# anuragranj/cc

Measured on NVIDIA H100. Metric: train-step triplets/sec at 256x832x6lvl, higher is better.
Workload: dtype f32

## Files before the change

### cc_b200/csrc/conv_tc.cu

```cuda
#include "conv.cuh"

#ifndef CCB_CPU_SIM

#include <cuda.h>
#include <cudaTypedefs.h>

namespace ccb {

constexpr int TC_M = 128;
constexpr int TC_NMAX = 128;
constexpr int TC_KC = 8;
constexpr int TC_MAX_STAGES = 4;
constexpr int TC_PRODUCERS = 128;
constexpr int TC_CONSUMER_WARPS = 8;
constexpr int TC_THREADS = TC_PRODUCERS + 32 * TC_CONSUMER_WARPS;
constexpr int TC_MAX_TAPS = 49;
constexpr int TC_PRODUCER_REGS = 72, TC_CONSUMER_REGS = 216;

struct TcArgs {
    CUtensorMap wmap;
    const float* x;
    const float* bias;
    const float* res;
    float* out;
// ... 43 lines not shown
    }
}
__device__ __forceinline__ void fence_proxy_async() { asm volatile("fence.proxy.async.shared::cta;" ::: "memory"); }
__device__ __forceinline__ void fence_barrier_init() { asm volatile("fence.mbarrier_init.release.cluster;" ::: "memory"); }
__device__ __forceinline__ void mbar_arrive_expect_tx(uint64_t* bar, uint32_t bytes) {
    asm volatile("mbarrier.arrive.expect_tx.shared::cta.b64 _, [%0], %1;" ::"r"(smem_u32(bar)), "r"(bytes) : "memory");
}
__device__ __forceinline__ void tma_load_3d(void* dst, const CUtensorMap* map, uint64_t* bar, int c0, int c1, int c2) {
    asm volatile(
        "cp.async.bulk.tensor.3d.shared::cluster.global.mbarrier::complete_tx::bytes [%0], [%1, {%3, %4, %5}], [%2];"
        ::"r"(smem_u32(dst)), "l"(map), "r"(smem_u32(bar)), "r"(c0), "r"(c1), "r"(c2)
        : "memory");
}
__device__ __forceinline__ void tma_prefetch_map(const CUtensorMap* map) {
    asm volatile("prefetch.tensormap [%0];" ::"l"(map) : "memory");
}
__device__ __forceinline__ void cp_async_4(uint32_t dst, const float* src, bool valid) {
    asm volatile("cp.async.ca.shared.global [%0], [%1], 4, %2;" ::"r"(dst), "l"(src), "r"(valid ? 4 : 0) : "memory");
}
__device__ __forceinline__ void cp_async_arrive(uint64_t* bar) {
    asm volatile("cp.async.mbarrier.arrive.noinc.shared::cta.b64 [%0];" ::"r"(smem_u32(bar)) : "memory");
}
__device__ __forceinline__ void cp_async_wait_all() { asm volatile("cp.async.wait_all;" ::: "memory"); }
__device__ __forceinline__ float tf32_hi(float x) {
    uint32_t r;
    asm("cvt.rna.tf32.f32 %0, %1;" : "=r"(r) : "f"(x));
    return __uint_as_float(r);
}

__device__ __forceinline__ uint64_t wg_desc(uint32_t saddr) {
    return (uint64_t)((saddr & 0x3FFFF) >> 4) | ((uint64_t)1 << 16) | ((uint64_t)(1024 >> 4) << 32) | ((uint64_t)1 << 62);
}
__device__ __forceinline__ void wg_fence() { asm volatile("wgmma.fence.sync.aligned;" ::: "memory"); }
__device__ __forceinline__ void wg_commit() { asm volatile("wgmma.commit_group.sync.aligned;" ::: "memory"); }
template <int PENDING>
__device__ __forceinline__ void wg_wait() { asm volatile("wgmma.wait_group.sync.aligned %0;" ::"n"(PENDING) : "memory"); }
template <int R>
__device__ __forceinline__ void wg_fence_regs(float (&d)[R]) {
#pragma unroll
    for (int i = 0; i < R; ++i) asm volatile("" : "+f"(d[i])::"memory");
}
template <int K, int R>
__device__ __forceinline__ void wg_fence_regs(uint32_t (&d)[K][R]) {
#pragma unroll
    for (int k = 0; k < K; ++k)
#pragma unroll
        for (int i = 0; i < R; ++i) asm volatile("" : "+r"(d[k][i])::"memory");
}

__device__ __forceinline__ void wgmma_tf32_n16(float (&d)[8], uint64_t da, uint64_t db) {
    asm volatile(
        "{\n\t.reg .pred p;\n\tsetp.ne.b32 p, 1, 0;\n\t"
        "wgmma.mma_async.sync.aligned.m64n16k8.f32.tf32.tf32 "
        "{%0, %1, %2, %3, %4, %5, %6, %7}, "
        "%8, %9, p, 1, 1;\n\t}"
        : "+f"(d[0]), "+f"(d[1]), "+f"(d[2]), "+f"(d[3]), "+f"(d[4]), "+f"(d[5]), "+f"(d[6]), "+f"(d[7])
        : "l"(da), "l"(db));
}
__device__ __forceinline__ void wgmma_tf32_n32(float (&d)[16], uint64_t da, uint64_t db) {
    asm volatile(
        "{\n\t.reg .pred p;\n\tsetp.ne.b32 p, 1, 0;\n\t"
        "wgmma.mma_async.sync.aligned.m64n32k8.f32.tf32.tf32 "
        "{%0, %1, %2, %3, %4, %5, %6, %7, %8, %9, %10, %11, %12, %13, %14, %15}, "
        "%16, %17, p, 1, 1;\n\t}"
        : "+f"(d[0]), "+f"(d[1]), "+f"(d[2]), "+f"(d[3]), "+f"(d[4]), "+f"(d[5]), "+f"(d[6]), "+f"(d[7]),
          "+f"(d[8]), "+f"(d[9]), "+f"(d[10]), "+f"(d[11]), "+f"(d[12]), "+f"(d[13]), "+f"(d[14]), "+f"(d[15])
        : "l"(da), "l"(db));
}
__device__ __forceinline__ void wgmma_tf32_n64(float (&d)[32], uint64_t da, uint64_t db) {
    asm volatile(
        "{\n\t.reg .pred p;\n\tsetp.ne.b32 p, 1, 0;\n\t"
        "wgmma.mma_async.sync.aligned.m64n64k8.f32.tf32.tf32 "
        "{%0, %1, %2, %3, %4, %5, %6, %7, %8, %9, %10, %11, %12, %13, %14, %15,"
        " %16, %17, %18, %19, %20, %21, %22, %23, %24, %25, %26, %27, %28, %29, %30, %31}, "
        "%32, %33, p, 1, 1;\n\t}"
        : "+f"(d[0]), "+f"(d[1]), "+f"(d[2]), "+f"(d[3]), "+f"(d[4]), "+f"(d[5]), "+f"(d[6]), "+f"(d[7]),
          "+f"(d[8]), "+f"(d[9]), "+f"(d[10]), "+f"(d[11]), "+f"(d[12]), "+f"(d[13]), "+f"(d[14]), "+f"(d[15]),
          "+f"(d[16]), "+f"(d[17]), "+f"(d[18]), "+f"(d[19]), "+f"(d[20]), "+f"(d[21]), "+f"(d[22]), "+f"(d[23]),
          "+f"(d[24]), "+f"(d[25]), "+f"(d[26]), "+f"(d[27]), "+f"(d[28]), "+f"(d[29]), "+f"(d[30]), "+f"(d[31])
        : "l"(da), "l"(db));
}
__device__ __forceinline__ void wgmma_tf32_n128(float (&d)[64], uint64_t da, uint64_t db) {
    asm volatile(
        "{\n\t.reg .pred p;\n\tsetp.ne.b32 p, 1, 0;\n\t"
        "wgmma.mma_async.sync.aligned.m64n128k8.f32.tf32.tf32 "
        "{%0, %1, %2, %3, %4, %5, %6, %7, %8, %9, %10, %11, %12, %13, %14, %15,"
        " %16, %17, %18, %19, %20, %21, %22, %23, %24, %25, %26, %27, %28, %29, %30, %31,"
        " %32, %33, %34, %35, %36, %37, %38, %39, %40, %41, %42, %43, %44, %45, %46, %47,"
        " %48, %49, %50, %51, %52, %53, %54, %55, %56, %57, %58, %59, %60, %61, %62, %63}, "
        "%64, %65, p, 1, 1;\n\t}"
        : "+f"(d[0]), "+f"(d[1]), "+f"(d[2]), "+f"(d[3]), "+f"(d[4]), "+f"(d[5]), "+f"(d[6]), "+f"(d[7]),
          "+f"(d[8]), "+f"(d[9]), "+f"(d[10]), "+f"(d[11]), "+f"(d[12]), "+f"(d[13]), "+f"(d[14]), "+f"(d[15]),
          "+f"(d[16]), "+f"(d[17]), "+f"(d[18]), "+f"(d[19]), "+f"(d[20]), "+f"(d[21]), "+f"(d[22]), "+f"(d[23]),
          "+f"(d[24]), "+f"(d[25]), "+f"(d[26]), "+f"(d[27]), "+f"(d[28]), "+f"(d[29]), "+f"(d[30]), "+f"(d[31]),
          "+f"(d[32]), "+f"(d[33]), "+f"(d[34]), "+f"(d[35]), "+f"(d[36]), "+f"(d[37]), "+f"(d[38]), "+f"(d[39]),
          "+f"(d[40]), "+f"(d[41]), "+f"(d[42]), "+f"(d[43]), "+f"(d[44]), "+f"(d[45]), "+f"(d[46]), "+f"(d[47]),
          "+f"(d[48]), "+f"(d[49]), "+f"(d[50]), "+f"(d[51]), "+f"(d[52]), "+f"(d[53]), "+f"(d[54]), "+f"(d[55]),
          "+f"(d[56]), "+f"(d[57]), "+f"(d[58]), "+f"(d[59]), "+f"(d[60]), "+f"(d[61]), "+f"(d[62]), "+f"(d[63])
        : "l"(da), "l"(db));
}
template <int NT>
__device__ __forceinline__ void wgmma_tf32(float (&d)[NT / 2], uint64_t da, uint64_t db) {
    if constexpr (NT == 16) wgmma_tf32_n16(d, da, db);
    else if constexpr (NT == 32) wgmma_tf32_n32(d, da, db);
    else if constexpr (NT == 64) wgmma_tf32_n64(d, da, db);
    else wgmma_tf32_n128(d, da, db);
}

__device__ __forceinline__ void wgmma_tf32_rs_n16(float (&d)[8], const uint32_t (&a)[4], uint64_t db) {
    asm volatile(
        "{\n\t.reg .pred p;\n\tsetp.ne.b32 p, 1, 0;\n\t"
        "wgmma.mma_async.sync.aligned.m64n16k8.f32.tf32.tf32 "
        "{%0, %1, %2, %3, %4, %5, %6, %7}, "
        "{%8, %9, %10, %11}, %12, p, 1, 1;\n\t}"
        : "+f"(d[0]), "+f"(d[1]), "+f"(d[2]), "+f"(d[3]), "+f"(d[4]), "+f"(d[5]), "+f"(d[6]), "+f"(d[7])
        : "r"(a[0]), "r"(a[1]), "r"(a[2]), "r"(a[3]), "l"(db));
}
__device__ __forceinline__ void wgmma_tf32_rs_n32(float (&d)[16], const uint32_t (&a)[4], uint64_t db) {
    asm volatile(
        "{\n\t.reg .pred p;\n\tsetp.ne.b32 p, 1, 0;\n\t"
        "wgmma.mma_async.sync.aligned.m64n32k8.f32.tf32.tf32 "
        "{%0, %1, %2, %3, %4, %5, %6, %7, %8, %9, %10, %11, %12, %13, %14, %15}, "
        "{%16, %17, %18, %19}, %20, p, 1, 1;\n\t}"
        : "+f"(d[0]), "+f"(d[1]), "+f"(d[2]), "+f"(d[3]), "+f"(d[4]), "+f"(d[5]), "+f"(d[6]), "+f"(d[7]),
          "+f"(d[8]), "+f"(d[9]), "+f"(d[10]), "+f"(d[11]), "+f"(d[12]), "+f"(d[13]), "+f"(d[14]), "+f"(d[15])
        : "r"(a[0]), "r"(a[1]), "r"(a[2]), "r"(a[3]), "l"(db));
}
__device__ __forceinline__ void wgmma_tf32_rs_n64(float (&d)[32], const uint32_t (&a)[4], uint64_t db) {
    asm volatile(
// ... 70 lines not shown
    __device__ __forceinline__ void publish(int s) const { fence_proxy_async(); mbar_arrive(&full[s]); }
};

__device__ __forceinline__ TcRing tc_ring(int depth, int b_tile_bytes, int full_arrivals) {
    CCB_PDL_TRIGGER();
    extern __shared__ __align__(1024) unsigned char smem_raw[];
    unsigned char* smem = smem_raw + ((1024u - (smem_u32(smem_raw) & 1023u)) & 1023u);
    const int stage_bytes = 2 * TC_TILE_BYTES + 2 * b_tile_bytes;
    uint64_t* full = (uint64_t*)(smem + depth * stage_bytes);
    const TcRing r = {smem, depth, stage_bytes, b_tile_bytes, full, full + TC_MAX_STAGES};
    if (threadIdx.x == 0) {
        for (int s = 0; s < depth; ++s) { mbar_init(&r.full[s], full_arrivals); mbar_init(&r.empty[s], TC_CONSUMER_WARPS); }
        fence_barrier_init();
    }
    __syncthreads();
    CCB_PDL_SYNC();
    return r;
}

__device__ __forceinline__ int tc_acc_row(int wg, int wq, int lane, int half) { return wg * 64 + wq * 16 + (lane >> 2) + half * 8; }
__device__ __forceinline__ int tc_acc_col(int lane, int i, int e) { return 8 * i + 2 * (lane & 3) + e; }
__device__ __forceinline__ int tc_acc_reg(int i, int half, int e) { return 4 * i + 2 * half + e; }

template <int NT>
__device__ __forceinline__ void tc_consume(const TcRing& ring, int nkt, int wg, int lane, float (&acc)[NT / 2]) {
    float part[NT / 2];
#pragma unroll
    for (int j = 0; j < NT / 2; ++j) acc[j] = 0.f;
    const uint32_t base = smem_u32(ring.smem);
    for (int it = 0; it < nkt; ++it) {
        const int s = it % ring.depth;
        mbar_wait(&ring.full[s], (it / ring.depth) & 1);
        const TcTiles<uint32_t> t = ring.tiles(base, s);
        const uint32_t a_hi = t.a_hi + wg * (TC_TILE_BYTES / 2), a_lo = t.a_lo + wg * (TC_TILE_BYTES / 2);
#pragma unroll
        for (int j = 0; j < NT / 2; ++j) part[j] = 0.f;
        wg_fence();
#pragma unroll
        for (int ks = 0; ks < TC_KC / 2; ++ks) {
            const uint32_t koff = (uint32_t)ks * 32u;
            wgmma_tf32<NT>(part, wg_desc(a_lo + koff), wg_desc(t.b_hi + koff));
            wgmma_tf32<NT>(part, wg_desc(a_hi + koff), wg_desc(t.b_lo + koff));
        }
#pragma unroll
        for (int ks = 0; ks < TC_KC / 2; ++ks) {
            const uint32_t koff = (uint32_t)ks * 32u;
            wgmma_tf32<NT>(part, wg_desc(a_hi + koff), wg_desc(t.b_hi + koff));
        }
        wg_commit();
        wg_wait<0>();
        wg_fence_regs(part);
        if (lane == 0) mbar_arrive(&ring.empty[s]);
#pragma unroll
        for (int j = 0; j < NT / 2; ++j) acc[j] += part[j];
    }
}

struct TcAFrag { uint32_t hi[TC_KC / 2][4], lo[TC_KC / 2][4]; };

__device__ __forceinline__ int tc_a_idx(int r, int k) { return k * TC_M + (r ^ (8 * (k & 3))); }
__device__ __forceinline__ int tc_a_off(int r0, int t) { return tc_a_idx(r0, t) * 4; }
__device__ __forceinline__ void tc_load_a(const unsigned char* tile, int off, float (&v)[2][8]) {
#pragma unroll
    for (int h = 0; h < 2; ++h)
#pragma unroll
        for (int j = 0; j < 8; ++j) v[h][j] = *(const float*)(tile + ((off ^ (32 * h)) + 2048 * j));
}
__device__ __forceinline__ void tc_split_a(const float (&v)[2][8], TcAFrag& f) {
#pragma unroll
    for (int ks = 0; ks < TC_KC / 2; ++ks)
#pragma unroll
        for (int i = 0; i < 4; ++i) {
            const float x = v[i & 1][2 * ks + (i >> 1)], h = tf32_hi(x);
            f.hi[ks][i] = __float_as_uint(h);
            f.lo[ks][i] = __float_as_uint(tf32_hi(x - h));
        }
}

template <int NT>
__device__ __forceinline__ void tc_consume_rs(const TcRing& ring, int g, int nkt, int wg, int wq, int lane, float (&acc)[NT / 2]) {
    constexpr bool split_ahead = NT < 128;
    float part[NT / 2];
#pragma unroll
    for (int j = 0; j < NT / 2; ++j) acc[j] = 0.f;
    const uint32_t base = smem_u32(ring.smem);
    const int a_off = tc_a_off(wg * 64 + wq * 16 + (lane >> 2), lane & 3);
    TcAFrag cur, nxt;
    float v[2][8];
    int s = g % ring.depth;
    uint32_t phase = (g / ring.depth) & 1;
    if constexpr (split_ahead) {
        if (nkt > 0) {
            mbar_wait(&ring.full[s], phase);
            tc_load_a(ring.tiles(ring.smem, s).a_hi, a_off, v);
            tc_split_a(v, cur);
        }
    }
    for (int it = 0; it < nkt; ++it) {
        if constexpr (!split_ahead) {
            mbar_wait(&ring.full[s], phase);
            tc_load_a(ring.tiles(ring.smem, s).a_hi, a_off, v);
            tc_split_a(v, cur);
        }
        const TcTiles<uint32_t> tl = ring.tiles(base, s);
#pragma unroll
        for (int j = 0; j < NT / 2; ++j) part[j] = 0.f;
        wg_fence();
#pragma unroll
        for (int ks = 0; ks < TC_KC / 2; ++ks) {
            const uint32_t koff = (uint32_t)ks * 32u;
            wgmma_tf32_rs<NT>(part, cur.lo[ks], wg_desc(tl.b_hi + koff));
            wgmma_tf32_rs<NT>(part, cur.hi[ks], wg_desc(tl.b_lo + koff));
        }
#pragma unroll
        for (int ks = 0; ks < TC_KC / 2; ++ks)
            wgmma_tf32_rs<NT>(part, cur.hi[ks], wg_desc(tl.b_hi + (uint32_t)ks * 32u));
        wg_commit();
        const int s1 = s + 1 == ring.depth ? 0 : s + 1;
        const uint32_t phase1 = phase ^ (s1 == 0);
        if constexpr (split_ahead) {
            if (it + 1 < nkt) {
                mbar_wait(&ring.full[s1], phase1);
                tc_load_a(ring.tiles(ring.smem, s1).a_hi, a_off, v);
                tc_split_a(v, nxt);
            }
        }
        wg_wait<0>();
        wg_fence_regs(part);
        wg_fence_regs(cur.hi);
        wg_fence_regs(cur.lo);
        if (lane == 0) mbar_arrive(&ring.empty[s]);
#pragma unroll
        for (int j = 0; j < NT / 2; ++j) acc[j] += part[j];
        if constexpr (split_ahead) cur = nxt;
        s = s1;
        phase = phase1;
    }
}

struct TcUnit { int m0, n0, z, kt_beg, nkt; };
__device__ __forceinline__ TcUnit tc_unit(const TcArgs& a, int u) {
    TcUnit w;
    w.m0 = (u % a.tiles_m) * TC_M;
    u /= a.tiles_m;
    w.n0 = (u % a.tiles_n) * TC_NMAX;
    w.z = u / a.tiles_n;
    w.kt_beg = w.z * a.kt_per_split;
    w.nkt = max(0, min(a.ktiles, w.kt_beg + a.kt_per_split) - w.kt_beg);
    return w;
}

template <int NT>
__global__ void __launch_bounds__(TC_THREADS, 1) conv_tc_kernel(const __grid_constant__ TcArgs a) {
    const TcRing ring = tc_ring(a.depth, a.b_tile_bytes, TC_PRODUCERS + 1);
    const int tid = threadIdx.x, warp = tid >> 5, lane = tid & 31;
    const long long HWin = (long long)a.Hin * a.Win;

    if (warp < TC_PRODUCERS / 32) {
        wg_regs_dec<TC_PRODUCER_REGS>();
        const int r = tid;
        const int cpt = a.cpad >> 2;
        const int nchunks = a.ntaps * cpt;
        if (r == 0) tma_prefetch_map(&a.wmap);
        int g = 0;
// ... 18 lines not shown
                if (r == 0) {
                    mbar_arrive_expect_tx(&ring.full[s], 2 * ring.b_tile_bytes);
                    tma_load_3d(t.b_hi, &a.wmap, &ring.full[s], kt * (TC_KC * 4), w.n0, 0);
                    tma_load_3d(t.b_lo, &a.wmap, &ring.full[s], kt * (TC_KC * 4), w.n0, 1);
                }
                const uint32_t at = smem_u32(t.a_hi);
                const int q0 = kt * TC_KC;
                const int tap0 = q0 / cpt, c40 = q0 - tap0 * cpt;
                if (c40 + TC_KC <= cpt) {
                    bool ok = mvalid && tap0 < a.ntaps;
                    int pix = 0;
                    if (ok) {
                        const int iy = iy0 + a.off_y[tap0], ix = ix0 + a.off_x[tap0];
                        ok = (iy >= 0) && (iy < a.Hin) && (ix >= 0) && (ix < a.Win);
                        pix = iy * a.Win + ix;
                    }
                    const float* p = ok ? xb + (long long)(c40 * 4) * HWin + pix : a.x;
                    const int nv = ok ? (a.Cin - c40 * 4) : 0;
#pragma unroll
                    for (int c = 0; c < TC_KC; ++c)
#pragma unroll
                        for (int j = 0; j < 4; ++j) {
                            const bool v = c * 4 + j < nv;
                            cp_async_4(at + 4 * tc_a_idx(r, 4 * c + j), v ? p + (c * 4 + j) * HWin : a.x, v);
                        }
                } else {
                    int q = q0, tap = tap0, c4 = c40;
#pragma unroll
                    for (int c = 0; c < TC_KC; ++c) {
                        const float* p = a.x;
                        int nv = 0;
                        if (mvalid && q < nchunks) {
                            const int iy = iy0 + a.off_y[tap], ix = ix0 + a.off_x[tap];
                            if (iy >= 0 && iy < a.Hin && ix >= 0 && ix < a.Win) {
                                p = xb + (long long)(c4 * 4) * HWin + (iy * a.Win + ix);
                                nv = a.Cin - c4 * 4;
                            }
                        }
#pragma unroll
                        for (int j = 0; j < 4; ++j) {
                            const bool v = j < nv;
                            cp_async_4(at + 4 * tc_a_idx(r, 4 * c + j), v ? p + j * HWin : a.x, v);
                        }
                        ++q;
                        if (++c4 == cpt) { c4 = 0; ++tap; }
                    }
                }
                cp_async_arrive(&ring.full[s]);
            }
        }
        cp_async_wait_all();
    } else {
        wg_regs_inc<TC_CONSUMER_REGS>();
        const int wg = (warp - TC_PRODUCERS / 32) >> 2, wq = warp & 3;
        const long long HWout = (long long)a.Hout * a.Wout;
        int g = 0;
        for (int u = blockIdx.x; u < a.units; u += gridDim.x) {
            const TcUnit w = tc_unit(a, u);
            const int ntile = min(TC_NMAX, a.Ntot - w.n0);
            float acc[NT / 2];
            tc_consume_rs<NT>(ring, g, w.nkt, wg, wq, lane, acc);
            g += w.nkt;
#pragma unroll
            for (int half = 0; half < 2; ++half) {
                const int em = w.m0 + tc_acc_row(wg, wq, lane, half);
                if (em >= a.M) continue;
                int hw = a.Hc * a.Wc;
                int eb = em / hw;
                int rem = em - eb * hw;
                int eoy = rem / a.Wc, eox = rem - eoy * a.Wc;
                const long long obase = (long long)eb * a.Ntot * HWout + (long long)(eoy * a.out_stride + a.out_oy) * a.Wout +
                                        (eox * a.out_stride + a.out_ox);
#pragma unroll
                for (int i = 0; i < NT / 8; ++i)
#pragma unroll
                    for (int e = 0; e < 2; ++e) {
                        const int nl = tc_acc_col(lane, i, e);
                        if (nl < ntile) {
                            float o = acc[tc_acc_reg(i, half, e)];
                            const int n = w.n0 + nl;
                            const long long off = obase + (long long)n * HWout;
                            if (a.splits > 1) {
                                a.partial[(long long)w.z * a.out_numel + off] = o;
                            } else {
// ... 9 lines not shown
}

static int roundup(int v, int m) { return (v + m - 1) / m * m; }
static int tc_kp(int ntaps, int Cc) { return ntaps > 0 ? roundup(ntaps * roundup(Cc, 4), TC_KC * 4) : TC_KC * 4; }

static void tc_geometry(int N, int& nt, int& b_tile_bytes, int& depth, int& smem) {
    const int ntile_max = N < TC_NMAX ? N : TC_NMAX;
    nt = 16;
    while (nt < ntile_max) nt <<= 1;
    b_tile_bytes = nt * 128;
    const int stage = 2 * TC_TILE_BYTES + 2 * b_tile_bytes;
    depth = (TC_SMEM_MAX - 2048) / stage;
    if (depth > TC_MAX_STAGES) depth = TC_MAX_STAGES;
    smem = depth * stage + 2048;
}

template <typename Args>
static int tc_launch_kernel(void (*const (&kfns)[4])(const Args), const Args& a, int nt, dim3 grid, int smem, cudaStream_t st,
                            const char* what) {
    auto kfn = kfns[nt == 16 ? 0 : nt == 32 ? 1 : nt == 64 ? 2 : 3];
    cudaFuncSetAttribute(kfn, cudaFuncAttributeMaxDynamicSharedMemorySize, TC_SMEM_MAX);
    CCB_LAUNCH(kfn, grid, dim3(TC_THREADS), smem, st, a);
    return check_launch(what);
}

static void (*const TC_FPROP_KERNELS[4])(const TcArgs) = {conv_tc_kernel<16>, conv_tc_kernel<32>, conv_tc_kernel<64>,
                                                          conv_tc_kernel<128>};

static int tc_weight_map(CUtensorMap* map, const float* wp, int N, int Kp, int nt) {
    static PFN_cuTensorMapEncodeTiled_v12000 encode = [] {
        void* fn = nullptr;
        cudaDriverEntryPointQueryResult q;
        if (cudaGetDriverEntryPointByVersion("cuTensorMapEncodeTiled", &fn, 12000, cudaEnableDefault, &q) != cudaSuccess ||
            q != cudaDriverEntryPointSuccess)
            fn = nullptr;
        return (PFN_cuTensorMapEncodeTiled_v12000)fn;
    }();
    CCB_REQUIRE(encode, CCB_ERR_LAUNCH, "conv_tc: the driver has no cuTensorMapEncodeTiled");
    const cuuint64_t dims[3] = {(cuuint64_t)Kp, (cuuint64_t)N, 2};
    const cuuint64_t strides[2] = {(cuuint64_t)Kp * sizeof(float), (cuuint64_t)N * Kp * sizeof(float)};
    const cuuint32_t box[3] = {TC_KC * 4, (cuuint32_t)nt, 1};
    const cuuint32_t estrides[3] = {1, 1, 1};
    const CUresult rc = encode(map, CU_TENSOR_MAP_DATA_TYPE_FLOAT32, 3, (void*)wp, dims, strides, box, estrides,
                               CU_TENSOR_MAP_INTERLEAVE_NONE, CU_TENSOR_MAP_SWIZZLE_128B, CU_TENSOR_MAP_L2_PROMOTION_L2_256B,
                               CU_TENSOR_MAP_FLOAT_OOB_FILL_NONE);
    CCB_REQUIRE(rc == CUDA_SUCCESS, CCB_ERR_LAUNCH, "conv_tc: cuTensorMapEncodeTiled failed (%d) for N %d Kp %d", (int)rc, N, Kp);
// ... 4 lines not shown
                     float* wp, float* partial, int splits, cudaStream_t st) {
    a.cpad = roundup(Cc, 4);
    a.Kp = tc_kp(a.ntaps, Cc);
    WPrepDesc p;
    memset(&p, 0, sizeof(p));
    p.w = w; p.wp = wp; p.N = N; p.Cc = Cc; p.KK = KK; p.ntaps = a.ntaps; p.Kp = a.Kp; p.mode = mode; p.Ci = Ci;
    p.layout = WPREP_TC; p.p0 = a.cpad;
    for (int t = 0; t < a.ntaps; ++t) p.tap_index[t] = tap_index[t];
    const float* wpp = nullptr;
    int rc = wprep_get(p, st, &wpp);
    if (rc) return rc;
    a.Ntot = N;
    a.splits = splits;
    a.ktiles = a.Kp / (TC_KC * 4);
    a.kt_per_split = cdiv(a.ktiles, splits);
    a.partial = partial;
    int nt, smem;
    tc_geometry(N, nt, a.b_tile_bytes, a.depth, smem);
    rc = tc_weight_map(&a.wmap, wpp, N, a.Kp, nt);
    if (rc) return rc;
    a.tiles_m = cdiv(a.M, TC_M);
    a.tiles_n = cdiv(N, TC_NMAX);
    a.units = a.tiles_m * a.tiles_n * splits;
    static int sms = [] {
        int dev = 0, n = 0;
        cudaGetDevice(&dev);
        cudaDeviceGetAttribute(&n, cudaDevAttrMultiProcessorCount, dev);
        return n > 0 ? n : NUM_SMS;
    }();
    return tc_launch_kernel(TC_FPROP_KERNELS, a, nt, dim3(a.units < sms ? a.units : sms), smem, st, "conv_tc");
}

struct TcWgradArgs {
    const float* x;
    const float* dy;
    float* out;
    int B, Ci, Hi, Wi, Co, Ho, Wo, kh, kw, stride, pad;
    int cpad, Mtot;
    int P;
    int ktiles, kt_per_split, splits;
    int depth, b_tile_bytes;
};

template <int NT>
__global__ void __launch_bounds__(TC_THREADS, 1) conv_tc_wgrad_kernel(const TcWgradArgs a) {
    const TcRing ring = tc_ring(a.depth, a.b_tile_bytes, TC_PRODUCERS);
    const int tid = threadIdx.x, warp = tid >> 5, lane = tid & 31;
    const int m0 = blockIdx.x * TC_M, n0 = blockIdx.y * TC_NMAX;
    const int ntile = min(TC_NMAX, a.Co - n0);
    const int kt_beg = blockIdx.z * a.kt_per_split;
    const int nkt = min(a.ktiles, kt_beg + a.kt_per_split) - kt_beg;
    const int KK = a.kh * a.kw;
    const int HWo = a.Ho * a.Wo, HWi = a.Hi * a.Wi;

    if (warp < TC_PRODUCERS / 32) {
        const int c = tid & 7, rbase = tid >> 3;
        int rowoff[8], dky[8], dkx[8];
        unsigned rvalid = 0;
#pragma unroll
        for (int j = 0; j < 8; ++j) {
            int m = m0 + rbase + 16 * j;
            rowoff[j] = 0; dky[j] = dkx[j] = 0;
            if (m < a.Mtot) {
                int tap = m / a.cpad, ci = m - tap * a.cpad;
                if (ci < a.Ci) {
                    int ky = tap / a.kw, kx = tap - ky * a.kw;
                    dky[j] = ky - a.pad; dkx[j] = kx - a.pad;
                    rowoff[j] = ci * HWi + dky[j] * a.Wi + dkx[j];
                    rvalid |= 1u << j;
                }
            }
        }
        for (int it = 0; it < nkt; ++it) {
            const int s = it % ring.depth;
            const int p0 = ((kt_beg + it) * TC_KC + c) * 4;
            const bool pvalid = p0 < a.P;
            int b = 0, oy = 0, ox0 = 0;
            if (pvalid) {
                b = p0 / HWo;
                int rem = p0 - b * HWo;
                oy = rem / a.Wo;
                ox0 = rem - oy * a.Wo;
            }
            const float* xpix = a.x + (long long)b * a.Ci * HWi + (oy * a.stride) * a.Wi + ox0 * a.stride;
            const int iyb = oy * a.stride, ixb = ox0 * a.stride;
            float av[8][4];
            float4 bv[8];
#pragma unroll
            for (int j = 0; j < 8; ++j) {
                av[j][0] = av[j][1] = av[j][2] = av[j][3] = 0.f;
                const int iy = iyb + dky[j], ix0 = ixb + dkx[j];
                if (pvalid && ((rvalid >> j) & 1u) && iy >= 0 && iy < a.Hi) {
                    const float* px = xpix + rowoff[j];
                    if (ix0 >= 0 && ix0 + 3 * a.stride < a.Wi) {
#pragma unroll
                        for (int e = 0; e < 4; ++e) av[j][e] = __ldg(px + e * a.stride);
                    } else {
#pragma unroll
                        for (int e = 0; e < 4; ++e) {
                            const int ix = ix0 + e * a.stride;
                            if (ix >= 0 && ix < a.Wi) av[j][e] = __ldg(px + e * a.stride);
                        }
                    }
                }
                bv[j] = make_float4(0.f, 0.f, 0.f, 0.f);
                const int n = rbase + 16 * j;
                if (pvalid && n < ntile)
                    bv[j] = __ldg((const float4*)(a.dy + ((long long)b * a.Co + n0 + n) * HWo + oy * a.Wo + ox0));
            }
            const TcTiles<unsigned char*> t = ring.acquire(it, s);
#pragma unroll
            for (int j = 0; j < 8; ++j) {
                const int r = rbase + 16 * j, idx = tile_idx(r, c);
                tc_split_store(t.a_hi, t.a_lo, idx, make_float4(av[j][0], av[j][1], av[j][2], av[j][3]));
                if (r < NT) tc_split_store(t.b_hi, t.b_lo, idx, bv[j]);
            }
            ring.publish(s);
        }
    } else {
        const int wg = (warp - TC_PRODUCERS / 32) >> 2, wq = warp & 3;
        float acc[NT / 2];
        tc_consume<NT>(ring, nkt, wg, lane, acc);
        float* outp = a.out + (long long)blockIdx.z * a.Co * a.Ci * KK;
#pragma unroll
        for (int half = 0; half < 2; ++half) {
            const int em = m0 + tc_acc_row(wg, wq, lane, half);
            if (em >= a.Mtot) continue;
            const int etap = em / a.cpad;
            const int eci = em - etap * a.cpad;
            if (eci >= a.Ci) continue;
#pragma unroll
            for (int i = 0; i < NT / 8; ++i)
#pragma unroll
                for (int e = 0; e < 2; ++e) {
                    const int nl = tc_acc_col(lane, i, e);
                    if (nl < ntile) outp[((long long)(n0 + nl) * a.Ci + eci) * KK + etap] = acc[tc_acc_reg(i, half, e)];
                }
        }
    }
}

static void (*const TC_WGRAD_KERNELS[4])(const TcWgradArgs) = {conv_tc_wgrad_kernel<16>, conv_tc_wgrad_kernel<32>,
                                                                conv_tc_wgrad_kernel<64>, conv_tc_wgrad_kernel<128>};

bool tc_supported(const ccb_conv_desc* d, int op) {
    if (d->kh != d->kw || d->kh * d->kw > TC_MAX_TAPS) return false;
    if (op == CCB_CONV_WGRAD) return (d->Wo % 4 == 0);
    return true;
}
bool tc_profitable(const ccb_conv_desc* d, int op) {
    if (!tc_supported(d, op)) return false;
    const long long M = (op == CCB_CONV_FPROP) ? (long long)d->B * d->Ho * d->Wo : (long long)d->B * d->Hi * d->Wi;
    const long long wsize = (long long)d->Ci * d->Co * d->kh * d->kw;
    return (M >= 128 && wsize >= 64) || (M >= 8 && wsize >= 65536);
}

int tc_plan(const ccb_conv_desc* d, int op, long long& panel_floats) {
    panel_floats = 0;
    if (op == CCB_CONV_WGRAD) {
        const int ktiles = cdiv(d->B * d->Ho * d->Wo, 32);
// ... 76 lines not shown
    if (splits > 1) {
        launch_splitk_reduce(partial, dx, bias, res, out_numel, splits, d->Hi * d->Wi, d->Ci, d->act, d->slope, st);
        return check_launch("conv_tc dgrad splitk reduce");
    }
    return CCB_OK;
}

int tc_wgrad(const ccb_conv_desc* d, const float* x, const float* dy, float* dw, float* partial, int splits, cudaStream_t st) {
    TcWgradArgs a;
    memset(&a, 0, sizeof(a));
    a.x = x; a.dy = dy;
    a.B = d->B; a.Ci = d->Ci; a.Hi = d->Hi; a.Wi = d->Wi; a.Co = d->Co; a.Ho = d->Ho; a.Wo = d->Wo;
    a.kh = d->kh; a.kw = d->kw; a.stride = d->stride; a.pad = d->pad;
    a.cpad = roundup(d->Ci, 4);
    a.Mtot = d->kh * d->kw * a.cpad;
    a.P = d->B * d->Ho * d->Wo;
    a.ktiles = cdiv(a.P, 32);
    a.kt_per_split = cdiv(a.ktiles, splits);
    a.splits = splits;
    a.out = splits > 1 ? partial : dw;
    const long long numel = (long long)d->Co * d->Ci * d->kh * d->kw;
    int nt, wsmem;
    tc_geometry(d->Co, nt, a.b_tile_bytes, a.depth, wsmem);
    dim3 grid(cdiv(a.Mtot, TC_M), cdiv(d->Co, TC_NMAX), a.splits);
    int rc = tc_launch_kernel(TC_WGRAD_KERNELS, a, nt, grid, wsmem, st, "conv_tc_wgrad");
    if (rc || a.splits == 1) return rc;
    launch_splitk_reduce(partial, dw, nullptr, nullptr, numel, splits, 1, 1, CCB_ACT_NONE, 0.f, st);
    return check_launch("conv_tc_wgrad_reduce");
}

}

extern "C" int ccb_debug_tc_plan(int N, int* out4) {
    if (N < 1 || !out4) return CCB_ERR_ARG;
    ccb::tc_geometry(N, out4[0], out4[1], out4[2], out4[3]);
    return CCB_OK;
}

#else

namespace ccb {
bool tc_supported(const ccb_conv_desc*, int) { return false; }
bool tc_profitable(const ccb_conv_desc*, int) { return false; }
int tc_plan(const ccb_conv_desc*, int, long long& panel_floats) { panel_floats = 0; return 1; }
int tc_fprop(const ccb_conv_desc*, const float*, const float*, const float*, const float*, float*, float*, float*, int,
             cudaStream_t) { return CCB_ERR_UNSUPPORTED; }
int tc_dgrad(const ccb_conv_desc*, const float*, const float*, const float*, const float*, float*, float*, float*, int,
             cudaStream_t) { return CCB_ERR_UNSUPPORTED; }
// ... 7 lines not shown
```

Measured before the change: 57.69.

## Restructure wgrad TC kernel: persistent grid, cp.async producers, register-A wgmma consumer

Rewrites the weight-gradient tensor-core kernel into a persistent, grid-strided kernel that iterates over work units. Producers now fill A via per-lane cp.async gathers into a swizzled row-major tile and stage dy via 16-byte cp.async, then split B into hi/lo a couple of stages later so loads stay in flight. Consumers switch from the shared-memory-descriptor wgmma path to the register-A path shared with fprop, with producer/consumer register reallocation. The aim is to hide global-load latency and cut launch and tail costs, at the price of more ring stages being held by the lag and a new requirement on ring depth.

```diff
diff --git a/cc_b200/csrc/conv_tc.cu b/cc_b200/csrc/conv_tc.cu
--- a/cc_b200/csrc/conv_tc.cu
+++ b/cc_b200/csrc/conv_tc.cu
@@ -89,6 +89,12 @@
     asm volatile("cp.async.mbarrier.arrive.noinc.shared::cta.b64 [%0];" ::"r"(smem_u32(bar)) : "memory");
 }
 __device__ __forceinline__ void cp_async_wait_all() { asm volatile("cp.async.wait_all;" ::: "memory"); }
+__device__ __forceinline__ void cp_async_16(uint32_t dst, const float* src, bool valid) {
+    asm volatile("cp.async.cg.shared.global [%0], [%1], 16, %2;" ::"r"(dst), "l"(src), "r"(valid ? 16 : 0) : "memory");
+}
+__device__ __forceinline__ void cp_async_commit() { asm volatile("cp.async.commit_group;" ::: "memory"); }
+template <int N>
+__device__ __forceinline__ void cp_async_wait() { asm volatile("cp.async.wait_group %0;" ::"n"(N) : "memory"); }
 __device__ __forceinline__ float tf32_hi(float x) {
     uint32_t r;
     asm("cvt.rna.tf32.f32 %0, %1;" : "=r"(r) : "f"(x));
@@ -113,65 +119,6 @@
     for (int k = 0; k < K; ++k)
 #pragma unroll
         for (int i = 0; i < R; ++i) asm volatile("" : "+r"(d[k][i])::"memory");
-}
-
-__device__ __forceinline__ void wgmma_tf32_n16(float (&d)[8], uint64_t da, uint64_t db) {
-    asm volatile(
-        "{\n\t.reg .pred p;\n\tsetp.ne.b32 p, 1, 0;\n\t"
-        "wgmma.mma_async.sync.aligned.m64n16k8.f32.tf32.tf32 "
-        "{%0, %1, %2, %3, %4, %5, %6, %7}, "
-        "%8, %9, p, 1, 1;\n\t}"
-        : "+f"(d[0]), "+f"(d[1]), "+f"(d[2]), "+f"(d[3]), "+f"(d[4]), "+f"(d[5]), "+f"(d[6]), "+f"(d[7])
-        : "l"(da), "l"(db));
-}
-__device__ __forceinline__ void wgmma_tf32_n32(float (&d)[16], uint64_t da, uint64_t db) {
-    asm volatile(
-        "{\n\t.reg .pred p;\n\tsetp.ne.b32 p, 1, 0;\n\t"
-        "wgmma.mma_async.sync.aligned.m64n32k8.f32.tf32.tf32 "
-        "{%0, %1, %2, %3, %4, %5, %6, %7, %8, %9, %10, %11, %12, %13, %14, %15}, "
-        "%16, %17, p, 1, 1;\n\t}"
-        : "+f"(d[0]), "+f"(d[1]), "+f"(d[2]), "+f"(d[3]), "+f"(d[4]), "+f"(d[5]), "+f"(d[6]), "+f"(d[7]),
-          "+f"(d[8]), "+f"(d[9]), "+f"(d[10]), "+f"(d[11]), "+f"(d[12]), "+f"(d[13]), "+f"(d[14]), "+f"(d[15])
-        : "l"(da), "l"(db));
-}
-__device__ __forceinline__ void wgmma_tf32_n64(float (&d)[32], uint64_t da, uint64_t db) {
-    asm volatile(
-        "{\n\t.reg .pred p;\n\tsetp.ne.b32 p, 1, 0;\n\t"
-        "wgmma.mma_async.sync.aligned.m64n64k8.f32.tf32.tf32 "
-        "{%0, %1, %2, %3, %4, %5, %6, %7, %8, %9, %10, %11, %12, %13, %14, %15,"
-        " %16, %17, %18, %19, %20, %21, %22, %23, %24, %25, %26, %27, %28, %29, %30, %31}, "
-        "%32, %33, p, 1, 1;\n\t}"
-        : "+f"(d[0]), "+f"(d[1]), "+f"(d[2]), "+f"(d[3]), "+f"(d[4]), "+f"(d[5]), "+f"(d[6]), "+f"(d[7]),
-          "+f"(d[8]), "+f"(d[9]), "+f"(d[10]), "+f"(d[11]), "+f"(d[12]), "+f"(d[13]), "+f"(d[14]), "+f"(d[15]),
-          "+f"(d[16]), "+f"(d[17]), "+f"(d[18]), "+f"(d[19]), "+f"(d[20]), "+f"(d[21]), "+f"(d[22]), "+f"(d[23]),
-          "+f"(d[24]), "+f"(d[25]), "+f"(d[26]), "+f"(d[27]), "+f"(d[28]), "+f"(d[29]), "+f"(d[30]), "+f"(d[31])
-        : "l"(da), "l"(db));
-}
-__device__ __forceinline__ void wgmma_tf32_n128(float (&d)[64], uint64_t da, uint64_t db) {
-    asm volatile(
-        "{\n\t.reg .pred p;\n\tsetp.ne.b32 p, 1, 0;\n\t"
-        "wgmma.mma_async.sync.aligned.m64n128k8.f32.tf32.tf32 "
-        "{%0, %1, %2, %3, %4, %5, %6, %7, %8, %9, %10, %11, %12, %13, %14, %15,"
-        " %16, %17, %18, %19, %20, %21, %22, %23, %24, %25, %26, %27, %28, %29, %30, %31,"
-        " %32, %33, %34, %35, %36, %37, %38, %39, %40, %41, %42, %43, %44, %45, %46, %47,"
-        " %48, %49, %50, %51, %52, %53, %54, %55, %56, %57, %58, %59, %60, %61, %62, %63}, "
-        "%64, %65, p, 1, 1;\n\t}"
-        : "+f"(d[0]), "+f"(d[1]), "+f"(d[2]), "+f"(d[3]), "+f"(d[4]), "+f"(d[5]), "+f"(d[6]), "+f"(d[7]),
-          "+f"(d[8]), "+f"(d[9]), "+f"(d[10]), "+f"(d[11]), "+f"(d[12]), "+f"(d[13]), "+f"(d[14]), "+f"(d[15]),
-          "+f"(d[16]), "+f"(d[17]), "+f"(d[18]), "+f"(d[19]), "+f"(d[20]), "+f"(d[21]), "+f"(d[22]), "+f"(d[23]),
-          "+f"(d[24]), "+f"(d[25]), "+f"(d[26]), "+f"(d[27]), "+f"(d[28]), "+f"(d[29]), "+f"(d[30]), "+f"(d[31]),
-          "+f"(d[32]), "+f"(d[33]), "+f"(d[34]), "+f"(d[35]), "+f"(d[36]), "+f"(d[37]), "+f"(d[38]), "+f"(d[39]),
-          "+f"(d[40]), "+f"(d[41]), "+f"(d[42]), "+f"(d[43]), "+f"(d[44]), "+f"(d[45]), "+f"(d[46]), "+f"(d[47]),
-          "+f"(d[48]), "+f"(d[49]), "+f"(d[50]), "+f"(d[51]), "+f"(d[52]), "+f"(d[53]), "+f"(d[54]), "+f"(d[55]),
-          "+f"(d[56]), "+f"(d[57]), "+f"(d[58]), "+f"(d[59]), "+f"(d[60]), "+f"(d[61]), "+f"(d[62]), "+f"(d[63])
-        : "l"(da), "l"(db));
-}
-template <int NT>
-__device__ __forceinline__ void wgmma_tf32(float (&d)[NT / 2], uint64_t da, uint64_t db) {
-    if constexpr (NT == 16) wgmma_tf32_n16(d, da, db);
-    else if constexpr (NT == 32) wgmma_tf32_n32(d, da, db);
-    else if constexpr (NT == 64) wgmma_tf32_n64(d, da, db);
-    else wgmma_tf32_n128(d, da, db);
 }
 
 __device__ __forceinline__ void wgmma_tf32_rs_n16(float (&d)[8], const uint32_t (&a)[4], uint64_t db) {
@@ -288,50 +235,30 @@
 __device__ __forceinline__ int tc_acc_col(int lane, int i, int e) { return 8 * i + 2 * (lane & 3) + e; }
 __device__ __forceinline__ int tc_acc_reg(int i, int half, int e) { return 4 * i + 2 * half + e; }
 
-template <int NT>
-__device__ __forceinline__ void tc_consume(const TcRing& ring, int nkt, int wg, int lane, float (&acc)[NT / 2]) {
-    float part[NT / 2];
-#pragma unroll
-    for (int j = 0; j < NT / 2; ++j) acc[j] = 0.f;
-    const uint32_t base = smem_u32(ring.smem);
-    for (int it = 0; it < nkt; ++it) {
-        const int s = it % ring.depth;
-        mbar_wait(&ring.full[s], (it / ring.depth) & 1);
-        const TcTiles<uint32_t> t = ring.tiles(base, s);
-        const uint32_t a_hi = t.a_hi + wg * (TC_TILE_BYTES / 2), a_lo = t.a_lo + wg * (TC_TILE_BYTES / 2);
-#pragma unroll
-        for (int j = 0; j < NT / 2; ++j) part[j] = 0.f;
-        wg_fence();
-#pragma unroll
-        for (int ks = 0; ks < TC_KC / 2; ++ks) {
-            const uint32_t koff = (uint32_t)ks * 32u;
-            wgmma_tf32<NT>(part, wg_desc(a_lo + koff), wg_desc(t.b_hi + koff));
-            wgmma_tf32<NT>(part, wg_desc(a_hi + koff), wg_desc(t.b_lo + koff));
-        }
-#pragma unroll
-        for (int ks = 0; ks < TC_KC / 2; ++ks) {
-            const uint32_t koff = (uint32_t)ks * 32u;
-            wgmma_tf32<NT>(part, wg_desc(a_hi + koff), wg_desc(t.b_hi + koff));
-        }
-        wg_commit();
-        wg_wait<0>();
-        wg_fence_regs(part);
-        if (lane == 0) mbar_arrive(&ring.empty[s]);
-#pragma unroll
-        for (int j = 0; j < NT / 2; ++j) acc[j] += part[j];
-    }
-}
-
 struct TcAFrag { uint32_t hi[TC_KC / 2][4], lo[TC_KC / 2][4]; };
 
-__device__ __forceinline__ int tc_a_idx(int r, int k) { return k * TC_M + (r ^ (8 * (k & 3))); }
-__device__ __forceinline__ int tc_a_off(int r0, int t) { return tc_a_idx(r0, t) * 4; }
-__device__ __forceinline__ void tc_load_a(const unsigned char* tile, int off, float (&v)[2][8]) {
-#pragma unroll
-    for (int h = 0; h < 2; ++h)
-#pragma unroll
-        for (int j = 0; j < 8; ++j) v[h][j] = *(const float*)(tile + ((off ^ (32 * h)) + 2048 * j));
-}
+struct TcAKMajor {
+    static __device__ __forceinline__ int idx(int r, int k) { return k * TC_M + (r ^ (8 * (k & 3))); }
+    static __device__ __forceinline__ int off(int r0, int t) { return idx(r0, t) * 4; }
+    static __device__ __forceinline__ void load(const unsigned char* tile, int off, float (&v)[2][8]) {
+#pragma unroll
+        for (int h = 0; h < 2; ++h)
+#pragma unroll
+            for (int j = 0; j < 8; ++j) v[h][j] = *(const float*)(tile + ((off ^ (32 * h)) + 2048 * j));
+    }
+};
+
+struct TcARowMajor {
+    static __device__ __forceinline__ int byte(int r, int k) { return 128 * r + ((4 * k) ^ (16 * (r & 7))); }
+    static __device__ __forceinline__ int off(int r0, int t) { return byte(r0, t); }
+    static __device__ __forceinline__ void load(const unsigned char* tile, int off, float (&v)[2][8]) {
+#pragma unroll
+        for (int h = 0; h < 2; ++h)
+#pragma unroll
+            for (int j = 0; j < 8; ++j) v[h][j] = *(const float*)(tile + ((off ^ (16 * j)) + 1024 * h));
+    }
+};
+
 __device__ __forceinline__ void tc_split_a(const float (&v)[2][8], TcAFrag& f) {
 #pragma unroll
     for (int ks = 0; ks < TC_KC / 2; ++ks)
@@ -343,14 +270,14 @@
         }
 }
 
-template <int NT>
+template <int NT, class AL>
 __device__ __forceinline__ void tc_consume_rs(const TcRing& ring, int g, int nkt, int wg, int wq, int lane, float (&acc)[NT / 2]) {
     constexpr bool split_ahead = NT < 128;
     float part[NT / 2];
 #pragma unroll
     for (int j = 0; j < NT / 2; ++j) acc[j] = 0.f;
     const uint32_t base = smem_u32(ring.smem);
-    const int a_off = tc_a_off(wg * 64 + wq * 16 + (lane >> 2), lane & 3);
+    const int a_off = AL::off(wg * 64 + wq * 16 + (lane >> 2), lane & 3);
     TcAFrag cur, nxt;
     float v[2][8];
     int s = g % ring.depth;
@@ -358,14 +285,14 @@
     if constexpr (split_ahead) {
         if (nkt > 0) {
             mbar_wait(&ring.full[s], phase);
-            tc_load_a(ring.tiles(ring.smem, s).a_hi, a_off, v);
+            AL::load(ring.tiles(ring.smem, s).a_hi, a_off, v);
             tc_split_a(v, cur);
         }
     }
     for (int it = 0; it < nkt; ++it) {
         if constexpr (!split_ahead) {
             mbar_wait(&ring.full[s], phase);
-            tc_load_a(ring.tiles(ring.smem, s).a_hi, a_off, v);
+            AL::load(ring.tiles(ring.smem, s).a_hi, a_off, v);
             tc_split_a(v, cur);
         }
         const TcTiles<uint32_t> tl = ring.tiles(base, s);
@@ -387,7 +314,7 @@
         if constexpr (split_ahead) {
             if (it + 1 < nkt) {
                 mbar_wait(&ring.full[s1], phase1);
-                tc_load_a(ring.tiles(ring.smem, s1).a_hi, a_off, v);
+                AL::load(ring.tiles(ring.smem, s1).a_hi, a_off, v);
                 tc_split_a(v, nxt);
             }
         }
@@ -405,7 +332,8 @@
 }
 
 struct TcUnit { int m0, n0, z, kt_beg, nkt; };
-__device__ __forceinline__ TcUnit tc_unit(const TcArgs& a, int u) {
+template <class Args>
+__device__ __forceinline__ TcUnit tc_unit(const Args& a, int u) {
     TcUnit w;
     w.m0 = (u % a.tiles_m) * TC_M;
     u /= a.tiles_m;
@@ -470,7 +398,7 @@
 #pragma unroll
                         for (int j = 0; j < 4; ++j) {
                             const bool v = c * 4 + j < nv;
-                            cp_async_4(at + 4 * tc_a_idx(r, 4 * c + j), v ? p + (c * 4 + j) * HWin : a.x, v);
+                            cp_async_4(at + 4 * TcAKMajor::idx(r, 4 * c + j), v ? p + (c * 4 + j) * HWin : a.x, v);
                         }
                 } else {
                     int q = q0, tap = tap0, c4 = c40;
@@ -488,7 +416,7 @@
 #pragma unroll
                         for (int j = 0; j < 4; ++j) {
                             const bool v = j < nv;
-                            cp_async_4(at + 4 * tc_a_idx(r, 4 * c + j), v ? p + j * HWin : a.x, v);
+                            cp_async_4(at + 4 * TcAKMajor::idx(r, 4 * c + j), v ? p + j * HWin : a.x, v);
                         }
                         ++q;
                         if (++c4 == cpt) { c4 = 0; ++tap; }
@@ -507,7 +435,7 @@
             const TcUnit w = tc_unit(a, u);
             const int ntile = min(TC_NMAX, a.Ntot - w.n0);
             float acc[NT / 2];
-            tc_consume_rs<NT>(ring, g, w.nkt, wg, wq, lane, acc);
+            tc_consume_rs<NT, TcAKMajor>(ring, g, w.nkt, wg, wq, lane, acc);
             g += w.nkt;
 #pragma unroll
             for (int half = 0; half < 2; ++half) {
@@ -563,6 +491,16 @@
     cudaFuncSetAttribute(kfn, cudaFuncAttributeMaxDynamicSharedMemorySize, TC_SMEM_MAX);
     CCB_LAUNCH(kfn, grid, dim3(TC_THREADS), smem, st, a);
     return check_launch(what);
+}
+
+static dim3 tc_grid(int units) {
+    static int sms = [] {
+        int dev = 0, n = 0;
+        cudaGetDevice(&dev);
+        cudaDeviceGetAttribute(&n, cudaDevAttrMultiProcessorCount, dev);
+        return n > 0 ? n : NUM_SMS;
+    }();
+    return dim3(units < sms ? units : sms);
 }
 
 static void (*const TC_FPROP_KERNELS[4])(const TcArgs) = {conv_tc_kernel<16>, conv_tc_kernel<32>, conv_tc_kernel<64>,
@@ -613,13 +551,7 @@
     a.tiles_m = cdiv(a.M, TC_M);
     a.tiles_n = cdiv(N, TC_NMAX);
     a.units = a.tiles_m * a.tiles_n * splits;
-    static int sms = [] {
-        int dev = 0, n = 0;
-        cudaGetDevice(&dev);
-        cudaDeviceGetAttribute(&n, cudaDevAttrMultiProcessorCount, dev);
-        return n > 0 ? n : NUM_SMS;
-    }();
-    return tc_launch_kernel(TC_FPROP_KERNELS, a, nt, dim3(a.units < sms ? a.units : sms), smem, st, "conv_tc");
+    return tc_launch_kernel(TC_FPROP_KERNELS, a, nt, tc_grid(a.units), smem, st, "conv_tc");
 }
 
 struct TcWgradArgs {
@@ -630,103 +562,160 @@
     int cpad, Mtot;
     int P;
     int ktiles, kt_per_split, splits;
+    int tiles_m, tiles_n, units;
     int depth, b_tile_bytes;
 };
 
+constexpr int TC_WGRAD_LAG = 2;
+
+template <int SEG>
+__device__ __forceinline__ void tc_wgrad_gather(const TcWgradArgs& a, uint32_t at, int lane, const float* xb, bool pv, int iyb,
+                                                int ixb, int tap, int ci, int ky, int kx) {
+    const long long HWi = (long long)a.Hi * a.Wi;
+#pragma unroll
+    for (int sg = 0; sg < 32 / SEG; ++sg) {
+        const int iy = iyb + ky, ix = ixb + kx;
+        const bool ok = pv && tap < a.kh * a.kw && (unsigned)iy < (unsigned)a.Hi && (unsigned)ix < (unsigned)a.Wi;
+        const float* src = ok ? xb + ci * HWi + (iy * a.Wi + ix) : a.x;
+        const int nv = ok ? a.Ci - ci : 0;
+#pragma unroll
+        for (int r = 0; r < SEG; ++r) {
+            const bool v = r < nv;
+            cp_async_4(at + TcARowMajor::byte(sg * SEG + r, lane), v ? src + r * HWi : a.x, v);
+        }
+        if ((ci += SEG) == a.cpad) {
+            ci = 0;
+            ++tap;
+            if (++kx == a.kw) { kx = 0; ++ky; }
+        }
+    }
+}
+
 template <int NT>
-__global__ void __launch_bounds__(TC_THREADS, 1) conv_tc_wgrad_kernel(const TcWgradArgs a) {
+__global__ void __launch_bounds__(TC_THREADS, 1) conv_tc_wgrad_kernel(const __grid_constant__ TcWgradArgs a) {
     const TcRing ring = tc_ring(a.depth, a.b_tile_bytes, TC_PRODUCERS);
     const int tid = threadIdx.x, warp = tid >> 5, lane = tid & 31;
-    const int m0 = blockIdx.x * TC_M, n0 = blockIdx.y * TC_NMAX;
-    const int ntile = min(TC_NMAX, a.Co - n0);
-    const int kt_beg = blockIdx.z * a.kt_per_split;
-    const int nkt = min(a.ktiles, kt_beg + a.kt_per_split) - kt_beg;
     const int KK = a.kh * a.kw;
     const int HWo = a.Ho * a.Wo, HWi = a.Hi * a.Wi;
 
     if (warp < TC_PRODUCERS / 32) {
-        const int c = tid & 7, rbase = tid >> 3;
-        int rowoff[8], dky[8], dkx[8];
-        unsigned rvalid = 0;
-#pragma unroll
-        for (int j = 0; j < 8; ++j) {
-            int m = m0 + rbase + 16 * j;
-            rowoff[j] = 0; dky[j] = dkx[j] = 0;
-            if (m < a.Mtot) {
-                int tap = m / a.cpad, ci = m - tap * a.cpad;
-                if (ci < a.Ci) {
-                    int ky = tap / a.kw, kx = tap - ky * a.kw;
-                    dky[j] = ky - a.pad; dkx[j] = kx - a.pad;
-                    rowoff[j] = ci * HWi + dky[j] * a.Wi + dkx[j];
-                    rvalid |= 1u << j;
+        wg_regs_dec<TC_PRODUCER_REGS>();
+        const int c = tid & 7, nb = tid >> 3;
+        auto split_b = [&](int g) {
+            const int s = g % ring.depth;
+            const TcTiles<unsigned char*> t = ring.tiles(ring.smem, s);
+#pragma unroll
+            for (int j = 0; j < NT / 16; ++j) {
+                const int n = nb + 16 * j;
+                tc_split_store(t.b_hi, t.b_lo, tile_idx(n, c), ((const float4*)t.a_lo)[n * TC_KC + c]);
+            }
+            ring.publish(s);
+        };
+        int g = 0;
+        for (int u = blockIdx.x; u < a.units; u += gridDim.x) {
+            const TcUnit w = tc_unit(a, u);
+            const int ntile = min(TC_NMAX, a.Co - w.n0);
+            const int mw = w.m0 + 32 * warp;
+            const int tap_w = mw / a.cpad, ci_w = mw - tap_w * a.cpad;
+            const int ky_w = tap_w / a.kw, kx_w = tap_w - ky_w * a.kw;
+            for (int it = 0; it < w.nkt; ++it, ++g) {
+                const int s = g % ring.depth;
+                const int kt = w.kt_beg + it;
+                const TcTiles<unsigned char*> t = ring.acquire(g, s);
+                const int p = kt * 32 + lane;
+                const bool pv = p < a.P;
+                int b = 0, oy = 0, ox = 0;
+                if (pv) {
+                    b = p / HWo;
+                    const int rem = p - b * HWo;
+                    oy = rem / a.Wo;
+                    ox = rem - oy * a.Wo;
+                }
+                const float* xb = a.x + (long long)b * a.Ci * HWi;
+                const int iyb = oy * a.stride - a.pad, ixb = ox * a.stride - a.pad;
+                const uint32_t at = smem_u32(t.a_hi) + 128 * 32 * warp;
+                if (ci_w + 32 <= a.cpad) {
+                    const int iy = iyb + ky_w, ix = ixb + kx_w;
+                    const bool ok = pv && tap_w < KK && (unsigned)iy < (unsigned)a.Hi && (unsigned)ix < (unsigned)a.Wi;
+                    const float* src = ok ? xb + (long long)ci_w * HWi + (iy * a.Wi + ix) : a.x;
+                    const int nv = ok ? a.Ci - ci_w : 0;
+#pragma unroll
+                    for (int i = 0; i < 32; ++i) {
+                        const bool v = i < nv;
+                        cp_async_4(at + TcARowMajor::byte(i, lane), v ? src + (long long)i * HWi : a.x, v);
+                    }
+                } else if (NT == 16 && a.cpad < 32) {
+                    const int seg = a.cpad & -a.cpad;
+                    if (seg == 16) tc_wgrad_gather<16>(a, at, lane, xb, pv, iyb, ixb, tap_w, ci_w, ky_w, kx_w);
+                    else if (seg == 8) tc_wgrad_gather<8>(a, at, lane, xb, pv, iyb, ixb, tap_w, ci_w, ky_w, kx_w);
+                    else tc_wgrad_gather<4>(a, at, lane, xb, pv, iyb, ixb, tap_w, ci_w, ky_w, kx_w);
+                } else {
+                    int tap = tap_w, ci = ci_w, ky = ky_w, kx = kx_w;
+                    for (int i = 0; i < 32;) {
+                        const int len = min(32 - i, a.cpad - ci);
+                        const int iy = iyb + ky, ix = ixb + kx;
+                        const bool ok = pv && tap < KK && (unsigned)iy < (unsigned)a.Hi && (unsigned)ix < (unsigned)a.Wi;
+                        const float* src = ok ? xb + (long long)ci * HWi + (iy * a.Wi + ix) : a.x;
+                        const int nv = ok ? a.Ci - ci : 0;
+                        for (int r = 0; r < len; ++r, ++i, src += HWi) {
+                            const bool v = r < nv;
+                            cp_async_4(at + TcARowMajor::byte(i, lane), v ? src : a.x, v);
+                        }
+                        ci = 0;
+                        ++tap;
+                        if (++kx == a.kw) { kx = 0; ++ky; }
+                    }
+                }
+                const int p4 = kt * 32 + 4 * c;
+                const bool bv = p4 < a.P;
+                int bb = 0, brem = 0;
+                if (bv) {
+                    bb = p4 / HWo;
+                    brem = p4 - bb * HWo;
+                }
+                const float* dyp = a.dy + ((long long)bb * a.Co + w.n0) * HWo + brem;
+                const uint32_t braw = smem_u32(t.a_lo);
+#pragma unroll
+                for (int j = 0; j < NT / 16; ++j) {
+                    const int n = nb + 16 * j;
+                    const bool v = bv && n < ntile;
+                    cp_async_16(braw + 16 * (n * TC_KC + c), v ? dyp + (long long)n * HWo : a.dy, v);
+                }
+                cp_async_commit();
+                if (g >= TC_WGRAD_LAG) {
+                    cp_async_wait<TC_WGRAD_LAG>();
+                    split_b(g - TC_WGRAD_LAG);
                 }
             }
         }
-        for (int it = 0; it < nkt; ++it) {
-            const int s = it % ring.depth;
-            const int p0 = ((kt_beg + it) * TC_KC + c) * 4;
-            const bool pvalid = p0 < a.P;
-            int b = 0, oy = 0, ox0 = 0;
-            if (pvalid) {
-                b = p0 / HWo;
-                int rem = p0 - b * HWo;
-                oy = rem / a.Wo;
-                ox0 = rem - oy * a.Wo;
+        cp_async_wait_all();
+        for (int gs = max(0, g - TC_WGRAD_LAG); gs < g; ++gs) split_b(gs);
+    } else {
+        wg_regs_inc<TC_CONSUMER_REGS>();
+        const int wg = (warp - TC_PRODUCERS / 32) >> 2, wq = warp & 3;
+        int g = 0;
+        for (int u = blockIdx.x; u < a.units; u += gridDim.x) {
+            const TcUnit w = tc_unit(a, u);
+            const int ntile = min(TC_NMAX, a.Co - w.n0);
+            float acc[NT / 2];
+            tc_consume_rs<NT, TcARowMajor>(ring, g, w.nkt, wg, wq, lane, acc);
+            g += w.nkt;
+            float* outp = a.out + (long long)w.z * a.Co * a.Ci * KK;
+#pragma unroll
+            for (int half = 0; half < 2; ++half) {
+                const int em = w.m0 + tc_acc_row(wg, wq, lane, half);
+                if (em >= a.Mtot) continue;
+                const int etap = em / a.cpad;
+                const int eci = em - etap * a.cpad;
+                if (eci >= a.Ci) continue;
+#pragma unroll
+                for (int i = 0; i < NT / 8; ++i)
+#pragma unroll
+                    for (int e = 0; e < 2; ++e) {
+                        const int nl = tc_acc_col(lane, i, e);
+                        if (nl < ntile) outp[((long long)(w.n0 + nl) * a.Ci + eci) * KK + etap] = acc[tc_acc_reg(i, half, e)];
+                    }
             }
-            const float* xpix = a.x + (long long)b * a.Ci * HWi + (oy * a.stride) * a.Wi + ox0 * a.stride;
-            const int iyb = oy * a.stride, ixb = ox0 * a.stride;
-            float av[8][4];
-            float4 bv[8];
-#pragma unroll
-            for (int j = 0; j < 8; ++j) {
-                av[j][0] = av[j][1] = av[j][2] = av[j][3] = 0.f;
-                const int iy = iyb + dky[j], ix0 = ixb + dkx[j];
-                if (pvalid && ((rvalid >> j) & 1u) && iy >= 0 && iy < a.Hi) {
-                    const float* px = xpix + rowoff[j];
-                    if (ix0 >= 0 && ix0 + 3 * a.stride < a.Wi) {
-#pragma unroll
-                        for (int e = 0; e < 4; ++e) av[j][e] = __ldg(px + e * a.stride);
-                    } else {
-#pragma unroll
-                        for (int e = 0; e < 4; ++e) {
-                            const int ix = ix0 + e * a.stride;
-                            if (ix >= 0 && ix < a.Wi) av[j][e] = __ldg(px + e * a.stride);
-                        }
-                    }
-                }
-                bv[j] = make_float4(0.f, 0.f, 0.f, 0.f);
-                const int n = rbase + 16 * j;
-                if (pvalid && n < ntile)
-                    bv[j] = __ldg((const float4*)(a.dy + ((long long)b * a.Co + n0 + n) * HWo + oy * a.Wo + ox0));
-            }
-            const TcTiles<unsigned char*> t = ring.acquire(it, s);
-#pragma unroll
-            for (int j = 0; j < 8; ++j) {
-                const int r = rbase + 16 * j, idx = tile_idx(r, c);
-                tc_split_store(t.a_hi, t.a_lo, idx, make_float4(av[j][0], av[j][1], av[j][2], av[j][3]));
-                if (r < NT) tc_split_store(t.b_hi, t.b_lo, idx, bv[j]);
-            }
-            ring.publish(s);
-        }
-    } else {
-        const int wg = (warp - TC_PRODUCERS / 32) >> 2, wq = warp & 3;
-        float acc[NT / 2];
-        tc_consume<NT>(ring, nkt, wg, lane, acc);
-        float* outp = a.out + (long long)blockIdx.z * a.Co * a.Ci * KK;
-#pragma unroll
-        for (int half = 0; half < 2; ++half) {
-            const int em = m0 + tc_acc_row(wg, wq, lane, half);
-            if (em >= a.Mtot) continue;
-            const int etap = em / a.cpad;
-            const int eci = em - etap * a.cpad;
-            if (eci >= a.Ci) continue;
-#pragma unroll
-            for (int i = 0; i < NT / 8; ++i)
-#pragma unroll
-                for (int e = 0; e < 2; ++e) {
-                    const int nl = tc_acc_col(lane, i, e);
-                    if (nl < ntile) outp[((long long)(n0 + nl) * a.Ci + eci) * KK + etap] = acc[tc_acc_reg(i, half, e)];
-                }
         }
     }
 }
@@ -849,8 +838,12 @@
     const long long numel = (long long)d->Co * d->Ci * d->kh * d->kw;
     int nt, wsmem;
     tc_geometry(d->Co, nt, a.b_tile_bytes, a.depth, wsmem);
-    dim3 grid(cdiv(a.Mtot, TC_M), cdiv(d->Co, TC_NMAX), a.splits);
-    int rc = tc_launch_kernel(TC_WGRAD_KERNELS, a, nt, grid, wsmem, st, "conv_tc_wgrad");
+    CCB_REQUIRE(TC_WGRAD_LAG <= a.depth - (nt < TC_NMAX ? 2 : 1), CCB_ERR_LAUNCH,
+                "conv_tc_wgrad: a ring of %d stages cannot hold the producers' lag of %d at N %d", a.depth, TC_WGRAD_LAG, nt);
+    a.tiles_m = cdiv(a.Mtot, TC_M);
+    a.tiles_n = cdiv(d->Co, TC_NMAX);
+    a.units = a.tiles_m * a.tiles_n * splits;
+    int rc = tc_launch_kernel(TC_WGRAD_KERNELS, a, nt, tc_grid(a.units), wsmem, st, "conv_tc_wgrad");
     if (rc || a.splits == 1) return rc;
     launch_splitk_reduce(partial, dw, nullptr, nullptr, numel, splits, 1, 1, CCB_ACT_NONE, 0.f, st);
     return check_launch("conv_tc_wgrad_reduce");
```

Result: faster. 58.83, median of 6 (+2.0%).
